# TGoldC/Motion-Planning-for-Autonomous-Driving-with-MPC

Measured on AMD Instinct MI355X. Metric: MPC steps/sec (N=30, nx=6 nu=2) at batch=4096, higher is better.
Workload: dtype f64; 1 GPU; N=30 nx=6 nu=2 bicycle lane-following, batch=4096/GPU, tol 1e-8; mode=converged, gpu=AMD Radeon Graphics

## Files before the change

### motion-planning-for-autonomous-driving-with-mpc_amd/csrc/mpc_solve_plan.h

```cpp
#pragma once
#include <algorithm>
#include <cctype>
#include <cstdlib>
#include <cstring>
#include <string>

#include "mpc_host_common.h"

namespace mpc {

struct Knobs {
    int pipeline, hybrid, hybrid_bx, hybrid_live, pipe_help, pipe_test_abort, pipe_xcd_mask;
    int rescue, rescue_wg, rescue_alone, loop_async, sync_spin, max_batch, friction_lb, bound_mask, big_wg, groups, poison;
    int timing;
    Knobs();
};
enum class KnobParse {
    ON,
    INT,
    FLAG,
    MASK,
    FRIC,
};
struct KnobDef { const char* name; int Knobs::*field; int dflt; KnobParse parse; };
inline constexpr KnobDef KNOBS[] = {
    {"pipeline", &Knobs::pipeline, 1, KnobParse::ON},           {"hybrid", &Knobs::hybrid, 1, KnobParse::INT},
    {"hybrid_bx", &Knobs::hybrid_bx, 0, KnobParse::INT},        {"hybrid_live", &Knobs::hybrid_live, -1, KnobParse::INT},
    {"pipe_help", &Knobs::pipe_help, -1, KnobParse::INT},       {"pipe_test_abort", &Knobs::pipe_test_abort, 0, KnobParse::FLAG},
    {"pipe_xcd_mask", &Knobs::pipe_xcd_mask, 0, KnobParse::MASK}, {"rescue", &Knobs::rescue, 1, KnobParse::ON},
    {"rescue_wg", &Knobs::rescue_wg, 1, KnobParse::INT},        {"rescue_alone", &Knobs::rescue_alone, 0, KnobParse::FLAG},
    {"loop_async", &Knobs::loop_async, 1, KnobParse::ON},       {"sync_spin", &Knobs::sync_spin, 1, KnobParse::ON},
    {"max_batch", &Knobs::max_batch, 0, KnobParse::INT},        {"friction_lb", &Knobs::friction_lb, 0, KnobParse::FRIC},
    {"bound_mask", &Knobs::bound_mask, 1, KnobParse::INT},      {"big_wg", &Knobs::big_wg, 0, KnobParse::FLAG},
    {"groups", &Knobs::groups, 0, KnobParse::INT},              {"poison", &Knobs::poison, 0, KnobParse::FLAG},
    {"timing", &Knobs::timing, 0, KnobParse::INT},
};
inline Knobs::Knobs() { for (const KnobDef& e : KNOBS) this->*e.field = e.dflt; }
inline const KnobDef* find_knob(const char* name) {
    for (const KnobDef& e : KNOBS) if (name && strcmp(name, e.name) == 0) return &e;
    return nullptr;
}
inline int set_knob(Knobs& k, const char* name, const char* value) {
    const KnobDef* e = find_knob(name);
    if (!e) return MPC_ERR_INVALID;
    int v = e->dflt;
    if (value) {
        const long iv = strtol(value, nullptr, 0);
        switch (e->parse) {
            case KnobParse::ON: v = value[0] != '0'; break;
            case KnobParse::INT: v = (int)iv; break;
            case KnobParse::FLAG: v = (value[0] == '\0' ? 1 : (int)iv) != 0; break;
            case KnobParse::MASK: v = (int)(uint32_t)strtoul(value, nullptr, 0); break;
            case KnobParse::FRIC: v = strcmp(value, "ipopt") == 0 ? 1 : strcmp(value, "nlp") == 0 ? 0 : (int)iv; break;
        }
    }
    k.*e->field = v;
    return MPC_OK;
}
// ... 206 lines not shown
```

### motion-planning-for-autonomous-driving-with-mpc_amd/csrc/mpc_stage_math.h

```cpp
#pragma once
#include <math.h>
#include <stdint.h>

#if defined(__HIPCC__)
#define MPC_HD __host__ __device__ __forceinline__
#else
#define MPC_HD inline
#endif

#if defined(__HIP_DEVICE_COMPILE__)
#define MPC_GLOBAL_AS __attribute__((address_space(1)))
#else
#define MPC_GLOBAL_AS
#endif
#define MPC_GP(ptr, idx) (((MPC_GLOBAL_AS __typeof__(*(ptr))*)(ptr))[(uint32_t)(idx)])

namespace mpc {

constexpr double MU_INIT = 0.1, KAPPA_EPS = 10.0, KAPPA_MU = 0.2, THETA_MU = 1.5, TAU_MIN = 0.99;
constexpr double KAPPA_1 = 1e-2, KAPPA_2 = 1e-2, S_MAX = 100.0, KAPPA_SIGMA = 1e10;
constexpr double GAMMA_THETA = 1e-5, GAMMA_PHI = 1e-8, LS_DELTA = 1.0, S_THETA = 1.1, S_PHI = 2.3;
constexpr double ETA_PHI = 1e-8, GAMMA_ALPHA = 0.05;
constexpr double DW_MIN = 1e-20, DW_0 = 1e-4, DW_MAX = 1e40, KW_MINUS = 1.0 / 3.0, KW_PLUS = 8.0, KW_PLUS_BAR = 100.0;
constexpr double SCALING_MAX_GRAD = 100.0;
// ... 185 lines not shown
#define MPC_KX(arr_, R, dk, e) (MB ? MPC_KI(P.M##arr_, R, dk, e) : MPC_K(P.arr_, R, dk, e))
#define MPC_ROWS(expr) [&](int e) -> decltype(auto) { return (expr); }
template <int CNT, class RefFn>
MPC_HD void ws_load_rows(RefFn ref, double* dst) {
#pragma unroll
    for (int i = 0; i + 1 < CNT; i += 2) MPC_LD2(ref(i), dst[i], dst[i + 1]);
    if (CNT & 1) dst[CNT - 1] = ref(CNT - 1);
}
template <int START, int CNT, class RefFn>
MPC_HD void ws_store_run(RefFn ref, const double* src) {
    constexpr int HEAD = START & 1;
    if (HEAD) ref(START) = src[0];
#pragma unroll
    for (int i = HEAD; i + 1 < CNT; i += 2) MPC_ST2(ref(START + i), src[i], src[i + 1]);
    if ((CNT - HEAD) & 1) ref(START + CNT - 1) = src[CNT - 1];
}
template <int CNT, class RefFn>
MPC_HD void ws_store_rows(RefFn ref, const double* src) {
#pragma unroll
    for (int i = 0; i + 1 < CNT; i += 2) MPC_ST2(ref(i), src[i], src[i + 1]);
    if (CNT & 1) ref(CNT - 1) = src[CNT - 1];
}

template <int NX>
struct Dim {
    static constexpr int NU = 2;
    static constexpr int NZ = NX + 2;
    static constexpr int NS = NX * (NX + 1) / 2;
    static constexpr int NH = NX + 5;
    MPC_HD static constexpr int hrow(int i, int j) {
        return i == j ? i : (i == 0 && j == 1) ? NX : (i == 0 && j == 4) ? NX + 1 : (i == 1 && j == 4) ? NX + 2
             : (i == 2 && j == 3) ? NX + 3 : (i == 3 && j == 4) ? NX + 4 : -1;
    }
    static constexpr int B_A = 0, B_RUU = 6, B_GU = 8, B_CN = 10, B_GX = 10 + NX, B_H = 10 + 2 * NX;
    static constexpr int NBLK = NH + 10 + 2 * NX;
    static constexpr int NPK = NS + NX;
    static constexpr int NKK = 2 * NX + 2;
    MPC_HD static constexpr int sidx(int i, int j) { return i * NX - i * (i - 1) / 2 + (j - i); }
};

struct Red0 { double gmax; };
struct Red1 { double a_pr, a_du, dphi; };
struct Red2 { double theta, fcost, logsum, bad; };
struct Red3 { double dual_inf, prim_inf, cmin, cmax, sum_mult, sum_z, theta, fcost, logsum, nan; };

MPC_HD Red0 red_neutral0() { return Red0{0.0}; }
// ... 1538 lines not shown
#pragma unroll
    for (int i = 0; i < NX; ++i) {
        if (i >= NE) { pv[i] = 0.0; continue; }
        double t = s.gx[i] + h[i] + g.G0[i] * kf0 + g.G1[i] * kf1;
        if (i == 2) t += a42 * h[4];
        if (i == 3) { t += a03 * h[0] + a13 * h[1] + a43 * h[4]; if (NE == 6) t += dt * h[NX - 1]; }
        if (i == 4) t += a04 * h[0] + a14 * h[1];
        pv[i] = t;
    }
}

template <int NX>
MPC_HD void ric_store_stage(const PRef& P, uint32_t bb, int k, const double* Ps, const double* pv, const RicGain<NX>& g) {
    using D = Dim<NX>;
    double kk[D::NKK], pk[D::NPK];
#pragma unroll
    for (int j = 0; j < NX; ++j) { kk[j] = g.K0[j]; kk[NX + j] = g.K1[j]; }
    kk[2 * NX] = g.kf0;
    kk[2 * NX + 1] = g.kf1;
#pragma unroll
    for (int i = 0; i < D::NS; ++i) pk[i] = Ps[i];
#pragma unroll
    for (int i = 0; i < NX; ++i) pk[D::NS + i] = pv[i];
    ws_store_rows<D::NKK>(MPC_ROWS(MPC_UK(P.KK, D::NKK, k, e)), kk);
    ws_store_rows<D::NPK>(MPC_ROWS(MPC_UK(P.PK, D::NPK, k, e)), pk);
}

template <int NX, int NE = NX, bool SYM = true>
MPC_HD bool riccati_backward_step(const PRef& P, uint32_t bb, int k, const RicStage<NX>& s, double delta, double hux0,
                                  double hux1, double* Ps, double* pv, bool sym_gk = false) {
    constexpr int NS = Dim<NX>::NS;
    double Pn[NS];
#pragma unroll
    for (int i = 0; i < NS; ++i) Pn[i] = Ps[i];
    RicGain<NX> g;
    if (!ric_matrix_step<NX, NE, SYM>(P, k, s, delta, hux0, hux1, Ps, g, sym_gk)) return false;
    ric_vector_step<NX, NE, SYM>(P, s, Pn, g, pv);
    ric_store_stage<NX>(P, bb, k, Ps, pv, g);
    return true;
}

template <int NX>
MPC_HD bool ric_bwd_any(const PRef& P, uint32_t bb, int k, const RicStage<NX>& s, double delta, double hux0, double hux1,
                        double* Ps, double* pv, bool sym_gk = false) {
    if (NX == 6 && P.dec_s && delta == 0.0) return riccati_backward_step<NX, (NX == 6 ? 5 : NX)>(P, bb, k, s, delta, hux0, hux1, Ps, pv, sym_gk);
    return riccati_backward_step<NX>(P, bb, k, s, delta, hux0, hux1, Ps, pv, sym_gk);
}

// ... 9 lines not shown
        f.K0[j] = MPC_UK(P.KK, D::NKK, k, j);
        f.K1[j] = MPC_UK(P.KK, D::NKK, k, NX + j);
        f.cn[j] = MPC_UK(P.BLK, D::NBLK, k, D::B_CN + j);
    }
    f.kf0 = MPC_UK(P.KK, D::NKK, k, 2 * NX);
    f.kf1 = MPC_UK(P.KK, D::NKK, k, 2 * NX + 1);
#pragma unroll
    for (int i = 0; i < 6; ++i) f.a[i] = MPC_UK(P.BLK, D::NBLK, k, D::B_A + i);
}

template <int NX>
MPC_HD void riccati_forward_step(const PRef& P, uint32_t bb, int k, const FwdStage<NX>& f, double* dx) {
    using D = Dim<NX>;
    const double dt = P.dt;
    double du0 = f.kf0, du1 = f.kf1;
#pragma unroll
    for (int j = 0; j < NX; ++j) { du0 += f.K0[j] * dx[j]; du1 += f.K1[j] * dx[j]; }
    {
        double dz[D::NZ];
        dz[0] = du0;
        dz[1] = du1;
#pragma unroll
        for (int i = 0; i < NX; ++i) dz[2 + i] = dx[i];
        ws_store_rows<D::NZ>(MPC_ROWS(MPC_UK(P.DZ, D::NZ, k, e)), dz);
    }
    double dn[NX];
#pragma unroll
    for (int i = 0; i < NX; ++i) dn[i] = dx[i] - f.cn[i];
    dn[0] += f.a[0] * dx[3] + f.a[1] * dx[4];
    dn[1] += f.a[2] * dx[3] + f.a[3] * dx[4];
    dn[2] += dt * du0;
    dn[3] += dt * du1;
    dn[4] += f.a[4] * dx[2] + f.a[5] * dx[3];
    if (NX == 6) dn[5] += dt * dx[3];
#pragma unroll
    for (int i = 0; i < NX; ++i) dx[i] = dn[i];
}

template <int NX>
MPC_HD void riccati_instance(const PRef& P, int b) {
    using D = Dim<NX>;
    constexpr int NS = D::NS;
    const int N = P.N;
    const uint32_t Bp = (uint32_t)P.Bp, bb = (uint32_t)b;
    if (MPC_U(P.ISC, (uint32_t)IS_STATUS) != ST_RUNNING) return;
    const double dt = P.dt;
    const double delta_last = MPC_U(P.SC, (uint32_t)SC_DLAST);
// ... 203 lines not shown
```

### motion-planning-for-autonomous-driving-with-mpc_amd/csrc/mpcgpu.hip

```cpp
#include <hip/hip_runtime.h>
#include <type_traits>

#include <algorithm>
#include <cctype>
#include <cstdio>
#include <cstdlib>
#include <cstring>
#include <new>
#include <string>
#include <vector>

#include "mpc_host_common.h"
#include "mpc_solve_plan.h"
#include "mpc_closed_loop.h"
#include "mpc_forces_qp.h"
#include "mpc_riccati_mfma.h"
#include "mpc_sens.h"

using namespace mpc;

namespace {

__device__ __forceinline__ void lds_barrier() {
    asm volatile("s_waitcnt lgkmcnt(0)\n\ts_barrier" ::: "memory");
// ... 289 lines not shown
template <int NX, bool INIT, int MAXT, uint32_t VM = 0xFFu>
__global__ void __launch_bounds__(MAXT, (INIT && MAXT <= 256) ? 2 : 1) k_stage(const Params Pk, const int n_mult, const int n_z, const int stash_rows) {
    const PRef P(Pk);
    extern __shared__ __attribute__((aligned(16))) double lds[];
    __shared__ int or_slots[2][8];
    uint32_t blk = blockIdx.x;
    if ((gridDim.x & 7u) == 0u) blk = (blk & 7u) * (gridDim.x >> 3) + (blk >> 3);
    const uint32_t b0 = (blk + (uint32_t)P.tile0 * (64u / (uint32_t)P.bx)) * (uint32_t)P.bx;
    const unsigned long long bits = (!INIT && P.tile_mask != nullptr) ? P.tile_mask[b0 >> 6] : ~0ull;
    stage_block<NX, INIT, MAXT, VM>(P, n_mult, n_z, stash_rows, b0, bits, lds, or_slots);
}

constexpr int32_t HO_IN_MB = 0x40000000;

template <int NCH>
__device__ __forceinline__ void wait_dma_behind(int stages_behind) {
    if (stages_behind >= 4 && 4 * NCH <= 63) asm volatile("s_waitcnt vmcnt(%0)" ::"n"(4 * NCH <= 63 ? 4 * NCH : 0) : "memory");
    else if (stages_behind >= 3 && 3 * NCH <= 63) asm volatile("s_waitcnt vmcnt(%0)" ::"n"(3 * NCH <= 63 ? 3 * NCH : 0) : "memory");
    else if (stages_behind >= 2) asm volatile("s_waitcnt vmcnt(%0)" ::"n"(2 * NCH) : "memory");
    else if (stages_behind == 1) asm volatile("s_waitcnt vmcnt(%0)" ::"n"(NCH) : "memory");
    else asm volatile("s_waitcnt vmcnt(0)" ::: "memory");
}

__device__ __forceinline__ void ho_lists(const PRef& P, const uint32_t bb, int32_t* ho_list, uint32_t* ho_count, const uint32_t* tile_word) {
#if defined(__HIP_DEVICE_COMPILE__)
    const int lane = threadIdx.x & 63;
    const bool active = (int)bb < P.B && (int32_t)MPC_U(P.ISC, (uint32_t)IS_STATUS) == ST_RUNNING;
    if (__ballot(active ? 1 : 0) == 0ull) return;
    const int32_t in_mb = (tile_word != nullptr && (__hip_atomic_load(tile_word + (bb >> 6), __ATOMIC_RELAXED, __HIP_MEMORY_SCOPE_AGENT) >> 31)) ? HO_IN_MB : 0;
    const double e0 = active ? (double)MPC_U(P.SC, (uint32_t)SC_E0) : 0.0;
    const int bucket = e0 >= 1e-3 ? 0 : e0 >= 1e-4 ? 1 : e0 >= 1e-5 ? 2 : 3;
    for (int q = 0; q < (int)HO_BUCKETS; ++q) {
        const unsigned long long mq = __ballot((active && bucket == q) ? 1 : 0);
        if (mq == 0ull) continue;
        uint32_t base = 0u;
        if (lane == 0) base = __hip_atomic_fetch_add(ho_count + q, (uint32_t)__popcll(mq), __ATOMIC_RELAXED, __HIP_MEMORY_SCOPE_AGENT);
        base = (uint32_t)__builtin_amdgcn_readfirstlane((int)base);
        if (active && bucket == q) ho_list[(uint32_t)q * (uint32_t)P.Bp + base + (uint32_t)__popcll(mq & ((1ull << lane) - 1ull))] = (int32_t)bb | in_mb;
    }
#endif
}

template <int NX>
__device__ __forceinline__ unsigned long long riccati_tile(const PRef& P, const uint32_t tile, char* smem, const bool stamp = true, const int handover_live = 0) {
#if defined(__HIP_DEVICE_COMPILE__)
    using D = Dim<NX>;
    constexpr int NS = D::NS;
    constexpr uint32_t BLK_BYTES = MPC_EV(D::NBLK) * 512u;
    constexpr int BLK_CHUNKS = (BLK_BYTES + 1023u) / 1024u;
    constexpr uint32_t SLOT = BLK_CHUNKS * 1024u;
    constexpr int KK_CHUNKS = (D::NKK * 512u + 1023u) / 1024u;
    constexpr int FWD_CHUNKS = KK_CHUNKS + 6;
    constexpr uint32_t FSLOT = FWD_CHUNKS * 1024u;
    static_assert(2 * BLK_CHUNKS <= 63 && RIC_DEPTH == 4 && 4 * FWD_CHUNKS <= 63 && RIC_DEPTH_F == 10, "vmcnt is a 6-bit counter");
    constexpr uint32_t RING_BYTES = (RIC_DEPTH * SLOT > RIC_DEPTH_F * FSLOT) ? RIC_DEPTH * SLOT : RIC_DEPTH_F * FSLOT;
    int* flag = reinterpret_cast<int*>(smem + RING_BYTES);
    const int wave = __builtin_amdgcn_readfirstlane((int)(threadIdx.x >> 6));
    const int lane = threadIdx.x & 63;
    const int b = (int)(tile * 64u) + lane;
    const uint32_t bb = (uint32_t)b;
    const int N = P.N;
    const bool active = (b < P.B) && ((int32_t)MPC_U(P.ISC, (uint32_t)IS_STATUS) == ST_RUNNING);
    const unsigned long long act_mask = __ballot(active ? 1 : 0);
    if (act_mask == 0ull) return 0ull;
    if (__popcll(act_mask) * 64 < handover_live * min(64, P.B - (int)(tile * 64u)) + 64) return 0ull;
#define RIC_STAMP(i) do { if (P.DBG && threadIdx.x == 0 && stamp) P.DBG[blockIdx.x * 16 + (i)] = __builtin_amdgcn_s_memtime(); } while (0)
    RIC_STAMP(0);
    const __amdgpu_buffer_rsrc_t rsrc = P.rws;
    const uint32_t tile_off = tile * P.tile_elems * 8u;
    const uint32_t blk_base = (uint32_t)(uintptr_t)P.BLK - (uint32_t)(uintptr_t)P.WS + tile_off;
    const uint32_t kk_base = (uint32_t)(uintptr_t)P.KK - (uint32_t)(uintptr_t)P.WS + tile_off;
    auto dma = [&](uint32_t src_, uint32_t dst_, int nchunks) {
        const uint32_t src = (uint32_t)__builtin_amdgcn_readfirstlane((int)src_), dst = (uint32_t)__builtin_amdgcn_readfirstlane((int)dst_);
#pragma unroll
        for (int c = 0; c < nchunks; ++c)
        {
            if (P.xcu) __builtin_amdgcn_raw_ptr_buffer_load_lds(rsrc, (lds_ptr_t)(smem + dst + (uint32_t)c * 1024u), 16, lane * 16, (int)(src + (uint32_t)c * 1024u), 0, MPC_AUX_SC1);
            else __builtin_amdgcn_raw_ptr_buffer_load_lds(rsrc, (lds_ptr_t)(smem + dst + (uint32_t)c * 1024u), 16, lane * 16, (int)(src + (uint32_t)c * 1024u), 0, 0);
        }
    };
    auto lds_r = [&](uint32_t off, uint32_t r) { return *reinterpret_cast<const double*>(smem + off + mpc_prow(r) * 8u + (uint32_t)lane * 16u); };
    auto read_stage = [&](uint32_t slot, RicStage<NX>& s) {
#pragma unroll
        for (int i = 0; i < NX; ++i) {
#pragma unroll
            for (int j = i; j < NX; ++j)
                s.H[D::sidx(i, j)] = (D::hrow(i, j) >= 0) ? lds_r(slot, D::B_H + (D::hrow(i, j) >= 0 ? D::hrow(i, j) : 0)) : 0.0;
        }
        s.ruu[0] = lds_r(slot, D::B_RUU);
        s.ruu[1] = lds_r(slot, D::B_RUU + 1);
#pragma unroll
        for (int i = 0; i < 6; ++i) s.a[i] = lds_r(slot, D::B_A + i);
#pragma unroll
        for (int i = 0; i < NX; ++i) { s.gx[i] = lds_r(slot, D::B_GX + i); s.cn[i] = lds_r(slot, D::B_CN + i); }
        s.gu[0] = lds_r(slot, D::B_GU);
        s.gu[1] = lds_r(slot, D::B_GU + 1);
    };
    double delta = 0.0, delta_last = 0.0, hux0 = 0.0, hux1 = 0.0;
    bool need = false, failed = false;
    if (wave == 0) {
        need = active;
        if (active) { delta_last = MPC_U(P.SC, (uint32_t)SC_DLAST); hux0 = MPC_U(P.SC, (uint32_t)SC_HUX0); hux1 = MPC_U(P.SC, (uint32_t)SC_HUX1); }
    }
    for (;;) {
        if (wave >= 2) {
            for (int t = 0; t <= N; ++t) lds_barrier();
        } else if (wave == 1) {
            for (int j = 0; j < RIC_DEPTH - 1 && j <= N; ++j) dma(blk_base + (uint32_t)(N - j) * BLK_BYTES, (uint32_t)j * SLOT, BLK_CHUNKS);
            for (int t = 0; t <= N; ++t) {
                const int k = N - t;
                wait_dma_behind<BLK_CHUNKS>(k < RIC_DEPTH - 2 ? k : RIC_DEPTH - 2);
                lds_barrier();
                const int kn = k - (RIC_DEPTH - 1);
                if (kn >= 0) dma(blk_base + (uint32_t)kn * BLK_BYTES, (uint32_t)((t + RIC_DEPTH - 1) % RIC_DEPTH) * SLOT, BLK_CHUNKS);
            }
        } else {
            bool ok = need;
            const bool sym = delta != 0.0 || delta_last != 0.0;
            auto sweep = [&](auto sym_tag, auto ne_tag) {
                constexpr bool SYM = decltype(sym_tag)::value;
                constexpr int NE = decltype(ne_tag)::value;
                double Ps[NS], pv[NX];
                for (int t = 0; t <= N; ++t) {
                    const int k = N - t;
                    if (t == 15) RIC_STAMP(3);
                    lds_barrier();
                    if (t == 15) RIC_STAMP(4);
                    RicStage<NX> s;
                    read_stage((uint32_t)(t % RIC_DEPTH) * SLOT, s);
                    if (t == 0) {
#pragma unroll
                        for (int i = 0; i < NS; ++i) Ps[i] = s.H[i];
#pragma unroll
                        for (int i = 0; i < NX; ++i) { Ps[D::sidx(i, i)] += delta; pv[i] = s.gx[i]; }
                        if (ok) {
                            double pk[D::NPK];
#pragma unroll
                            for (int i = 0; i < NS; ++i) pk[i] = Ps[i];
#pragma unroll
                            for (int i = 0; i < NX; ++i) pk[NS + i] = pv[i];
                            ws_store_rows<D::NPK>(MPC_ROWS(MPC_UK(P.PK, D::NPK, N, e)), pk);
                        }
                    } else if (ok) {
                        ok = riccati_backward_step<NX, NE, SYM>(P, bb, k, s, delta, hux0, hux1, Ps, pv, SYM && sym);
                    }
                    if (t == 15) RIC_STAMP(5);
                }
            };
            if (__any(sym ? 1 : 0)) sweep(std::true_type{}, std::integral_constant<int, NX>{});
            else if (NX == 6 && P.dec_s) sweep(std::false_type{}, std::integral_constant<int, (NX == 6 ? 5 : NX)>{});
            else sweep(std::false_type{}, std::integral_constant<int, NX>{});
            if (need && ok) need = false;
            else if (need) {
                if (delta == 0.0) delta = (delta_last == 0.0) ? DW_0 : fmax(DW_MIN, KW_MINUS * delta_last);
                else delta *= (delta_last == 0.0) ? KW_PLUS_BAR : KW_PLUS;
                if (delta > DW_MAX) { need = false; failed = true; }
            }
            const int again = __any(need ? 1 : 0);
            asm volatile("s_waitcnt vmcnt(0)" ::: "memory");
            if (lane == 0) *flag = again;
        }
        lds_barrier();
        const int again = lds_uniform(*flag);
        lds_barrier();
        if (!again) break;
    }
    RIC_STAMP(1);
    const bool go = (wave == 0) && active && !failed;
    if (wave >= 3) {
        for (int k = 0; k < N; ++k) lds_barrier();
    } else if (wave >= 1) {
        const int par = wave - 1;
        auto dma_fwd = [&](int k, uint32_t dst) {
            dma(kk_base + (uint32_t)k * (D::NKK * 512u), dst, KK_CHUNKS);
            static_assert(D::B_A % 2 == 0 && D::B_CN % 2 == 0 && D::NKK % 2 == 0, "sub-blocks copied on their own start on a row-pair boundary");
            dma(blk_base + (uint32_t)k * BLK_BYTES + D::B_A * 512u, dst + KK_CHUNKS * 1024u, 3);
            dma(blk_base + (uint32_t)k * BLK_BYTES + D::B_CN * 512u, dst + (KK_CHUNKS + 3) * 1024u, 3);
        };
        for (int j = par; j < RIC_DEPTH_F - 1 && j < N; j += 2) dma_fwd(j, (uint32_t)j * FSLOT);
        for (int k = 0; k < N; ++k) {
            if ((k & 1) == par) {
                const int last = (N - 1 < k + RIC_DEPTH_F - 2) ? N - 1 : k + RIC_DEPTH_F - 2;
                wait_dma_behind<FWD_CHUNKS>((last - k) >> 1);
            }
            lds_barrier();
            const int kn = k + RIC_DEPTH_F - 1;
            if (kn < N && (kn & 1) == par) dma_fwd(kn, (uint32_t)(kn % RIC_DEPTH_F) * FSLOT);
        }
    } else {
        if (active && failed) MPC_U(P.ISC, (uint32_t)IS_STATUS) = P.emit ? ST_SWEEP_FAILED : -7;
        if (go) {
            if (delta > 0.0) MPC_U(P.SC, (uint32_t)SC_DLAST) = delta;
            MPC_U(P.SC, (uint32_t)SC_DELTA) = delta;
        }
        double dx[NX];
#pragma unroll
        for (int i = 0; i < NX; ++i) dx[i] = go ? -(double)MPC_U(P.SC, (uint32_t)(SC_C0 + i)) : 0.0;
        for (int k = 0; k < N; ++k) {
            const uint32_t slot = (uint32_t)(k % RIC_DEPTH_F) * FSLOT;
            if (k == 15) RIC_STAMP(6);
            lds_barrier();
            if (k == 15) RIC_STAMP(7);
            if (k == 0) RIC_STAMP(9);
            FwdStage<NX> f;
#pragma unroll
            for (int j = 0; j < NX; ++j) {
                f.K0[j] = lds_r(slot, (uint32_t)j);
                f.K1[j] = lds_r(slot, (uint32_t)(NX + j));
                f.cn[j] = lds_r(slot + (KK_CHUNKS + 3) * 1024u, (uint32_t)j);
            }
            f.kf0 = lds_r(slot, (uint32_t)(2 * NX));
            f.kf1 = lds_r(slot, (uint32_t)(2 * NX + 1));
#pragma unroll
            for (int i = 0; i < 6; ++i) f.a[i] = lds_r(slot + KK_CHUNKS * 1024u, (uint32_t)i);
            riccati_forward_step<NX>(P, bb, k, f, dx);
            if (k == 15) RIC_STAMP(8);
        }
        if (go) {
            double dz[D::NZ];
            dz[0] = 0.0;
            dz[1] = 0.0;
#pragma unroll
            for (int i = 0; i < NX; ++i) dz[2 + i] = dx[i];
            ws_store_rows<D::NZ>(MPC_ROWS(MPC_UK(P.DZ, D::NZ, N, e)), dz);
        }
    }
    RIC_STAMP(2);
#undef RIC_STAMP
    return act_mask;
#else
    return 0ull;
#endif
}

template <int NX>
__global__ void __launch_bounds__(192) k_riccati(const Params Pk) {
    const PRef P(Pk);
    extern __shared__ __attribute__((aligned(16))) char smem[];
    const uint32_t tile = blockIdx.x + (uint32_t)P.tile0;
    const unsigned long long act_mask = riccati_tile<NX>(P, tile, smem);
    if (P.tile_mask != nullptr && threadIdx.x == 0) P.tile_mask[tile] = act_mask;
}

struct PipeArgs {
    uint32_t* ctl;
    uint32_t ntiles;
    uint32_t xcd_mask;
    uint32_t n_ric;
    uint32_t cap;
    uint32_t items;
    uint32_t handover;
    int32_t* ho_list;
    uint32_t flags;
};
constexpr uint32_t PIPE_EXIT = 0xFFFFFFFFu;
constexpr unsigned long long PIPE_SPIN_LIMIT = 5000000ull;
#ifndef MPC_PIPE_SLEEP
#define MPC_PIPE_SLEEP 8
#endif

__device__ __forceinline__ void pipe_acquire() {
#if defined(__HIP_DEVICE_COMPILE__)
    __builtin_amdgcn_fence(__ATOMIC_ACQUIRE, "workgroup");
// ... 69 lines not shown
                if (t == 0) {
                    uint32_t ok = 1u;
                    const uint32_t need = A.items * round;
                    const unsigned long long t0 = wall_clock64();
                    while (pipe_ld(stage_done + tile) < need) {
                        if (pipe_ld(abort_w)) { ok = 0u; break; }
                        if (wall_clock64() - t0 > PIPE_SPIN_LIMIT) {
                            pipe_st(abort_w + 28, (tile << 16) | (round & 0xFFFFu)); pipe_st(abort_w + 29, pipe_ld(stage_done + tile)); pipe_st(abort_w + 31, (uint32_t)(wall_clock64() - t0));
                            const unsigned long long t1 = wall_clock64();
                            while (wall_clock64() - t1 < 100000ull) __builtin_amdgcn_s_sleep(8);
                            pipe_st(abort_w + 30, pipe_ld(stage_done + tile));
                            pipe_st(abort_w, 2u); ok = 0u; break;
                        }
                        __builtin_amdgcn_s_sleep(MPC_PIPE_SLEEP);
                    }
                    waited += wall_clock64() - t0;
                    pipe_acquire();
                    asm volatile("s_waitcnt vmcnt(0)" ::: "memory");
                    sh_word[1] = ok;
                }
                lds_barrier();
                if (lds_uniform(sh_word[1]) == 0u) return;
                PIPE_STAMP(12);
                const unsigned long long mask = riccati_tile<NX>(P, tile, reinterpret_cast<char*>(lds), n_pass == 5u, (int)A.handover);
                if (mask == 0ull) {
                    fin |= 1u << j;
                    if (t == 0) {
                        if (round > 0u && P.mbw_live > 0 && __popcll(__hip_atomic_load(P.tile_mask + tile, __ATOMIC_RELAXED, __HIP_MEMORY_SCOPE_AGENT)) <= P.mbw_live)
                        {   __hip_atomic_fetch_or(stage_done + tile, 0x80000000u, __ATOMIC_RELAXED, __HIP_MEMORY_SCOPE_AGENT);
                            asm volatile("s_waitcnt vmcnt(0)" ::: "memory");
                        }
                        atomicMax(A.ctl + PIPE_ABORT + 1, round);
                        pipe_add(X + 48, 1u);
                    }
                } else if (t < 64) {
                    if (t == 0) __hip_atomic_store(P.tile_mask + tile, mask, __ATOMIC_RELAXED, __HIP_MEMORY_SCOPE_AGENT);
                    asm volatile("s_waitcnt vmcnt(0)" ::: "memory");
                    if (t == 0) {
                        const uint32_t tk = pipe_add(X + 32, A.items);
                        for (uint32_t q = 0; q < A.items; ++q)
                            __hip_atomic_store(slots + ((tk + q) & (A.cap - 1u)), ((unsigned long long)(tk + q + 1u) << 32) | (unsigned long long)((tile << 8) | q),
                                               __ATOMIC_RELAXED, __HIP_MEMORY_SCOPE_AGENT);
                    }
                }
                PIPE_STAMP(13);
                ++n_pass;
                lds_barrier();
                if constexpr (helper) if (mask != 0ull) {
                    if (t == 0) {
                        uint32_t item = PIPE_EXIT;
                        unsigned long long bits = 0ull;
                        uint32_t jn = j, rn = round;
                        do { if (++jn == n_own) { jn = 0u; ++rn; } } while (((fin >> jn) & 1u) && jn != j);
                        const uint32_t tile_n = (slot + jn * n_ric) * n_xcd + xcd;
                        if (pipe_ld(stage_done + tile_n) < A.items * rn) {
                            uint32_t hd = pipe_ld(X + 16);
                            bool got = false;
                            while ((int32_t)(pipe_ld(X + 32) - hd) > 0) {
                                uint32_t seen = hd;
                                if (__hip_atomic_compare_exchange_strong(X + 16, &seen, hd + 1u, __ATOMIC_RELAXED, __ATOMIC_RELAXED, __HIP_MEMORY_SCOPE_AGENT)) { got = true; break; }
                                hd = seen;
                            }
                            if (got) {
                                const unsigned long long* sl = slots + (hd & (A.cap - 1u));
                                const unsigned long long t0 = wall_clock64();
                                for (;;) {
                                    const unsigned long long v = __hip_atomic_load(sl, __ATOMIC_RELAXED, __HIP_MEMORY_SCOPE_AGENT);
                                    if ((uint32_t)(v >> 32) == hd + 1u) { item = (uint32_t)v; break; }
                                    if (pipe_ld(abort_w)) break;
                                    if (wall_clock64() - t0 > PIPE_SPIN_LIMIT) { pipe_st(abort_w + 28, hd); pipe_st(abort_w + 29, pipe_ld(X + 32)); pipe_st(abort_w + 31, (uint32_t)(wall_clock64() - t0)); pipe_st(abort_w, 3u); break; }
// ... 1524 lines not shown
    N_SCRATCH
};

struct mpc_handle {
    HostProblem hp;
    std::string err;
    int device = 0;
    size_t cap_Bp = 0;
    bool ws_mailbox = false;
    double* d_ws = nullptr;
    int32_t* d_iws = nullptr;
    double *d_LB = nullptr, *d_UB = nullptr;
    unsigned long long* d_tile_mask = nullptr;
    double* d_state = nullptr;
    size_t cap_state = 0;
    size_t tile_mask_cap = 0;
    uint32_t* d_pipe = nullptr;
    int pipe_flip = 0;
    size_t pipe_clean[2] = {0, 0};
    size_t pipe_words = 0;
    uint32_t* h_pipe = nullptr;
    bool pipe_disabled = false;
    int pipe_aborts = 0;
    static constexpr int PIPE_ABORTS_MAX = 3;
    int last_mode = 0;
    int32_t* d_counter = nullptr;
    int32_t* h_counter = nullptr;
    hipEvent_t ev_poll[4][2] = {};
    size_t cap_io = 0;
    double *d_x0 = nullptr, *d_p = nullptr, *d_xout = nullptr, *d_kkt = nullptr;
    int32_t *d_status = nullptr, *d_iters = nullptr;
    hipStream_t own_stream = nullptr;
    hipStream_t sub_stream[MAX_GROUPS] = {nullptr, nullptr, nullptr, nullptr};
    hipEvent_t ev_fork = nullptr, ev_join[MAX_GROUPS] = {nullptr, nullptr, nullptr, nullptr};
    bool profiling = false;
    bool prof_span = false;
    double prof[6] = {0, 0, 0, 0, 0, 0};
    double res_prof[8] = {0, 0, 0, 0, 0, 0, 0, 0};
    double pipe_prof[8] = {0, 0, 0, 0, 0, 0, 0, 0};
    int n_cu = 256;
    uint32_t xcd_mask = 0xFFu;
    std::vector<hipEvent_t> ev_pool;
    uint32_t* d_fail = nullptr;
    bool async_loop = false;
    bool async_ok = false;
    uint32_t* h_fail = nullptr;
// ... 177 lines not shown
    return MPC_OK;
}

int mpc_set_profiling(mpc_handle* h, int32_t enable) {
    if (!h) return MPC_ERR_INVALID;
    h->profiling = enable != 0;
    h->prof_span = enable == 2;
    return MPC_OK;
}

int mpc_set_option(mpc_handle* h, const char* name, const char* value) {
    if (!h || !name) return MPC_ERR_INVALID;
    const int rc = set_knob(h->knobs, name, value);
    if (rc) h->err = std::string("unknown option (or a value this build does not support): ") + name;
    else apply_fric_literal(h->hp, h->knobs.friction_lb);
    return rc;
}

int mpc_get_option(const mpc_handle* h, const char* name, int64_t* value) {
    if (!h || !name || !value) return MPC_ERR_INVALID;
    long v = 0;
    if (std::string(name) == "pipe_disabled") { *value = h->pipe_disabled ? 1 : 0; return MPC_OK; }
    if (std::string(name) == "pipe_aborts") { *value = h->pipe_aborts; return MPC_OK; }
    const int rc = get_knob(h->knobs, name, &v);
    if (rc == MPC_OK) *value = (int64_t)v;
    return rc;
}

int mpc_last_rescued(const mpc_handle* h) { return h ? h->rescued_last : MPC_ERR_INVALID; }

int mpc_get_pipeline_profile(const mpc_handle* h, double out[8]) {
    if (!h || !out) return MPC_ERR_INVALID;
    for (int i = 0; i < 8; ++i) out[i] = h->pipe_prof[i];
    return MPC_OK;
}

int mpc_get_resident_profile(const mpc_handle* h, double out[8]) {
    if (!h || !out) return MPC_ERR_INVALID;
    for (int i = 0; i < 8; ++i) out[i] = h->res_prof[i];
    return MPC_OK;
}

int mpc_measure_copy_bandwidth(mpc_handle* h, size_t bytes, int32_t reps, double* gbs) {
    if (!h || !gbs || reps < 1 || bytes < (1u << 20)) return MPC_ERR_INVALID;
    HIP_TRY(h, hipSetDevice(h->device));
    const size_t n = bytes / 16;
// ... 440 lines not shown
            h->async_ok = true;
            return MPC_OK;
        }
        HIP_TRY(h, wait_stream(h, stream));
        h->h_fail[0] = h->h_pipe[14];
        for (int q = 0; q < 4; ++q) h->h_fail[2 + q] = h->h_pipe[16 + q];
        if (h->resc_ran && !in_rescue) h->rescued_last = (int)h->h_pipe[20];
        report_wg_trace(d_wtrace, n_wtrace);
        if (P.DBG) {
            rc = report_wg_timing(h, P.DBG, pl.wg_grid);
            if (rc) return rc;
            P.DBG = nullptr;
        }
        piped = true;
        it = (int)h->h_fail[2];
        h->res_prof[1] = 1; h->res_prof[2] = it; h->res_prof[3] = pl.wg_grid; h->res_prof[4] = h->h_fail[3]; h->res_prof[5] = h->h_fail[4]; h->res_prof[6] = h->h_fail[5];
    } else if (pl.pipe_path) {
        PipeArgs A;
        A.ntiles = (uint32_t)ntiles;
        A.n_ric = (uint32_t)pl.n_ric;
        A.xcd_mask = pl.xcd_mask;
        A.items = 64u / (uint32_t)bx;
        A.cap = pl.pipe_cap;
        A.flags = kn.pipe_test_abort ? 2u : 0u;
        A.handover = (uint32_t)hand;
        A.ho_list = nullptr;
        if (hand > 0) {
            A.ho_list = static_cast<int32_t*>(scratch_get(h, SCR_HO_LIST, (size_t)HO_BUCKETS * Bp * sizeof(int32_t)));
            if (!A.ho_list) { h->err = "out of device memory"; return MPC_ERR_HIP; }
        }
        A.ctl = ctl;
        unsigned long long* d_pdbg = nullptr;
        if (pl.pipe_timing) {
            HIP_TRY(h, hipMalloc(&t_pdbg.p, sizeof(unsigned long long) * 16 * (size_t)h->n_cu));
            d_pdbg = t_pdbg.as<unsigned long long>();
            HIP_TRY(h, hipMemsetAsync(d_pdbg, 0, sizeof(unsigned long long) * 16 * (size_t)h->n_cu, stream));
            P.DBG = d_pdbg;
        }
        prof.next(3, stream);
        P.mbw_live = pl.mbw_live;
        const size_t lds_pipe = std::max(pl.lds_bytes, pl.ric_lds);
        if (pl.pipe_help) hipLaunchKernelGGL((k_pipeline<NX, 2, true>), dim3(h->n_cu), dim3(threads), lds_pipe, stream, P, A, h->hp.n_mult, h->hp.n_z, stash_rows);
        else if (pl.masked) hipLaunchKernelGGL((k_pipeline<NX, 2>), dim3(h->n_cu), dim3(threads), lds_pipe, stream, P, A, h->hp.n_mult, h->hp.n_z, stash_rows);
        else hipLaunchKernelGGL((k_pipeline<NX, false>), dim3(h->n_cu), dim3(threads), lds_pipe, stream, P, A, h->hp.n_mult, h->hp.n_z, stash_rows);
        if (hand <= 0) prof.end(stream);
        if (hand > 0) {
            if (!h->prof_span) prof.next(5, stream);
            wg_list = A.ho_list; wg_list_n = ctl + PIPE_HO;
            launch_wg((const uint32_t*)(ctl + PIPE_ABORT), ctl + PIPE_WG, h->async_loop ? nullptr : ctl + PIPE_ABORT);
        }
        prof.end(stream);
        if (h->async_loop) {
            hipLaunchKernelGGL(k_loop_sticky, dim3(1), dim3(1), 0, stream, (const uint32_t*)(ctl + PIPE_ABORT), h->d_fail + 1);
            HIP_TRY(h, hipGetLastError());
            h->async_ok = true;
            h->last_mode = 1;
            return MPC_OK;
        }
        if (hand <= 0) HIP_TRY(h, hipMemcpyAsync(h->h_pipe, ctl + PIPE_ABORT, PIPE_FIN_WORDS * sizeof(uint32_t), hipMemcpyDeviceToHost, stream));
        HIP_TRY(h, wait_stream(h, stream));
        h->h_fail[0] = h->h_pipe[14];
        report_wg_trace(d_wtrace, n_wtrace);
        for (int q = 0; q < 4; ++q) h->h_fail[2 + q] = h->h_pipe[16 + q];
        if (h->resc_ran && !in_rescue) h->rescued_last = (int)h->h_pipe[20];
        if (hand > 0) {
            h->res_prof[1] = 1; h->res_prof[2] = h->h_fail[2]; h->res_prof[3] = pl.wg_grid;
            h->res_prof[4] = h->h_fail[3]; h->res_prof[5] = h->h_fail[4]; h->res_prof[6] = h->h_fail[5];
        }
        if (h->h_pipe[0] != 0u) {
            h->pipe_disabled = true;
            h->resc_in_kernel = h->resc_ran = false;
            fprintf(stderr, "[mpcgpu] single-launch pipeline abandoned (bounded wait expired: code %u, %u / %u, a millisecond later %u, waited %u ticks); re-running with one launch per kernel\n",
                    h->h_pipe[0], h->h_pipe[28], h->h_pipe[29], h->h_pipe[30], h->h_pipe[31]);
            report_arrivals(ctl, ntiles, A.items);
            const int rc_again = solve_dev_impl<NX>(h, B, d_x0, d_p, d_obst, d_x_out, d_status, d_iters, d_kkt, stream, trace, trace_rows, n_it_out, in_rescue);
            if (++h->pipe_aborts < mpc_handle::PIPE_ABORTS_MAX) h->pipe_disabled = false;
            return rc_again;
        }
        P.DBG = nullptr;
        if (d_pdbg) { rc = report_pipe_timing(h, d_pdbg); if (rc) return rc; }
        piped = true;
        h->last_mode = 1;
        it = (int)h->h_pipe[1];
        const unsigned long long* st64 = reinterpret_cast<const unsigned long long*>(h->h_pipe + 2);
        h->pipe_prof[1] = 1; h->pipe_prof[2] = it;
        h->pipe_prof[3] = (double)st64[0] * 1e-5; h->pipe_prof[4] = (double)st64[1] * 1e-5; h->pipe_prof[5] = (double)st64[2] * 1e-5;
        h->pipe_prof[6] = (double)st64[3]; h->pipe_prof[7] = (double)h->h_pipe[12] + 1e-3 * (double)h->h_pipe[13];
    }
    if (!piped) {
        if (!h->async_loop) HIP_TRY(h, hipMemsetAsync(h->d_fail, 0, sizeof(uint32_t), stream));
        if (pl.polled) HIP_TRY(h, hipMemsetAsync(h->d_counter, 0, sizeof(int32_t) * MAX_GROUPS * MAX_POLL_IT, stream));
        if (G > 1) {
            HIP_TRY(h, hipEventRecord(h->ev_fork, stream));
// ... 754 lines not shown
```

Baseline: 5.328 million MPC steps/s.

## Replace per-stage workgroup barriers in Riccati sweeps with LDS progress counters

Removes the lock-step lds_barrier calls between the DMA loader waves and the compute wave in the backward and forward Riccati sweeps. In their place each wave publishes progress words in LDS and waits on them with a bounded spin, so idle waves no longer take part in the barriers. It also switches the workspace row stores to raw buffer stores with immediate offsets. The bounded wait adds an abort path, reported through the existing pipeline-abandon mechanism, and a test knob that forces it to expire; the risks are spin overhead and spurious timeouts.

Result: slower. 4.585 million MPC steps/s (-13.9%).

```diff
diff --git a/motion-planning-for-autonomous-driving-with-mpc_amd/csrc/mpc_solve_plan.h b/motion-planning-for-autonomous-driving-with-mpc_amd/csrc/mpc_solve_plan.h
--- a/motion-planning-for-autonomous-driving-with-mpc_amd/csrc/mpc_solve_plan.h
+++ b/motion-planning-for-autonomous-driving-with-mpc_amd/csrc/mpc_solve_plan.h
@@ -10,7 +10,7 @@
 namespace mpc {
 
 struct Knobs {
-    int pipeline, hybrid, hybrid_bx, hybrid_live, pipe_help, pipe_test_abort, pipe_xcd_mask;
+    int pipeline, hybrid, hybrid_bx, hybrid_live, pipe_help, pipe_test_abort, pipe_test_expire, pipe_xcd_mask;
     int rescue, rescue_wg, rescue_alone, loop_async, sync_spin, max_batch, friction_lb, bound_mask, big_wg, groups, poison;
     int timing;
     Knobs();
@@ -33,7 +33,7 @@
     {"max_batch", &Knobs::max_batch, 0, KnobParse::INT},        {"friction_lb", &Knobs::friction_lb, 0, KnobParse::FRIC},
     {"bound_mask", &Knobs::bound_mask, 1, KnobParse::INT},      {"big_wg", &Knobs::big_wg, 0, KnobParse::FLAG},
     {"groups", &Knobs::groups, 0, KnobParse::INT},              {"poison", &Knobs::poison, 0, KnobParse::FLAG},
-    {"timing", &Knobs::timing, 0, KnobParse::INT},
+    {"timing", &Knobs::timing, 0, KnobParse::INT},              {"pipe_test_expire", &Knobs::pipe_test_expire, 0, KnobParse::FLAG},
 };
 inline Knobs::Knobs() { for (const KnobDef& e : KNOBS) this->*e.field = e.dflt; }
 inline const KnobDef* find_knob(const char* name) {
diff --git a/motion-planning-for-autonomous-driving-with-mpc_amd/csrc/mpc_stage_math.h b/motion-planning-for-autonomous-driving-with-mpc_amd/csrc/mpc_stage_math.h
--- a/motion-planning-for-autonomous-driving-with-mpc_amd/csrc/mpc_stage_math.h
+++ b/motion-planning-for-autonomous-driving-with-mpc_amd/csrc/mpc_stage_math.h
@@ -231,6 +231,32 @@
     if (CNT & 1) ref(CNT - 1) = src[CNT - 1];
 }
 
+#if defined(__HIP_DEVICE_COMPILE__)
+template <int CNT, class RefFn>
+__device__ __forceinline__ void ws_store_rows_imm(RefFn ref, const double* src) {
+    const WsRefD r0 = ref(0);
+    const __amdgpu_buffer_rsrc_t d = r0.P.rws;
+    const uint32_t uni = (uint32_t)mpc_uni(r0.aoff + r0.uoff);
+#pragma unroll
+    for (int g = 0; g < CNT; g += 8) {
+        uint32_t base = r0.voff + (uint32_t)mpc_uni(uni + (uint32_t)g * 512u);
+        asm volatile("" : "+v"(base));
+#pragma unroll
+        for (int i = g; i < g + 8 && i < CNT; i += 2) {
+            if (i + 1 < CNT) {
+                const mpc_v2u a = __builtin_bit_cast(mpc_v2u, src[i]), b = __builtin_bit_cast(mpc_v2u, src[i + 1]);
+                __builtin_amdgcn_raw_buffer_store_b128(mpc_v4u{a.x, a.y, b.x, b.y}, d, (int)(base + (uint32_t)(i - g) * 512u), 0, 0);
+            } else {
+                __builtin_amdgcn_raw_buffer_store_b64(__builtin_bit_cast(mpc_v2u, src[i]), d, (int)(base + (uint32_t)(i - g) * 512u), 0, 0);
+            }
+        }
+    }
+}
+#else
+template <int CNT, class RefFn>
+MPC_HD void ws_store_rows_imm(RefFn ref, const double* src) { ws_store_rows<CNT>(ref, src); }
+#endif
+
 template <int NX>
 struct Dim {
     static constexpr int NU = 2;
@@ -1815,8 +1841,8 @@
     for (int i = 0; i < D::NS; ++i) pk[i] = Ps[i];
 #pragma unroll
     for (int i = 0; i < NX; ++i) pk[D::NS + i] = pv[i];
-    ws_store_rows<D::NKK>(MPC_ROWS(MPC_UK(P.KK, D::NKK, k, e)), kk);
-    ws_store_rows<D::NPK>(MPC_ROWS(MPC_UK(P.PK, D::NPK, k, e)), pk);
+    ws_store_rows_imm<D::NKK>(MPC_ROWS(MPC_UK(P.KK, D::NKK, k, e)), kk);
+    ws_store_rows_imm<D::NPK>(MPC_ROWS(MPC_UK(P.PK, D::NPK, k, e)), pk);
 }
 
 template <int NX, int NE = NX, bool SYM = true>
@@ -1872,7 +1898,7 @@
         dz[1] = du1;
 #pragma unroll
         for (int i = 0; i < NX; ++i) dz[2 + i] = dx[i];
-        ws_store_rows<D::NZ>(MPC_ROWS(MPC_UK(P.DZ, D::NZ, k, e)), dz);
+        ws_store_rows_imm<D::NZ>(MPC_ROWS(MPC_UK(P.DZ, D::NZ, k, e)), dz);
     }
     double dn[NX];
 #pragma unroll
diff --git a/motion-planning-for-autonomous-driving-with-mpc_amd/csrc/mpcgpu.hip b/motion-planning-for-autonomous-driving-with-mpc_amd/csrc/mpcgpu.hip
--- a/motion-planning-for-autonomous-driving-with-mpc_amd/csrc/mpcgpu.hip
+++ b/motion-planning-for-autonomous-driving-with-mpc_amd/csrc/mpcgpu.hip
@@ -335,6 +335,33 @@
     else asm volatile("s_waitcnt vmcnt(0)" ::: "memory");
 }
 
+constexpr int RIC_W_LD = 0, RIC_W_CP = 2, RIC_W_QUIT = 3, RIC_WORDS = 4;
+constexpr unsigned long long RIC_SPIN_LIMIT = 5000000ull;
+enum : int { RIC_QUIT_BWD = 1, RIC_QUIT_FWD = 2, RIC_QUIT_LOADER = 3, RIC_QUIT_TEST = 4 };
+__device__ __forceinline__ int ric_peek(const int* w) { return *reinterpret_cast<const volatile int*>(w); }
+__device__ __forceinline__ void ric_publish(int* w, const int v) {
+    asm volatile("" ::: "memory");
+    if ((threadIdx.x & 63) == 0) *reinterpret_cast<volatile int*>(w) = v;
+}
+__device__ __forceinline__ bool ric_wait(const int* w, const int need, const int seen, int* quit, const int code, const bool expire_now = false) {
+    bool ok = true;
+    if (lds_uniform(seen) < need || expire_now) {
+        const unsigned long long t0 = wall_clock64();
+        for (;;) {
+            if (!expire_now && lds_uniform(ric_peek(w)) >= need) break;
+            if (lds_uniform(ric_peek(quit)) != 0) { ok = false; break; }
+            if (expire_now || wall_clock64() - t0 > RIC_SPIN_LIMIT) {
+                if ((threadIdx.x & 63) == 0) *reinterpret_cast<volatile int*>(quit) = expire_now ? (int)RIC_QUIT_TEST : code;
+                ok = false;
+                break;
+            }
+            __builtin_amdgcn_s_sleep(1);
+        }
+    }
+    asm volatile("" ::: "memory");
+    return ok;
+}
+
 __device__ __forceinline__ void ho_lists(const PRef& P, const uint32_t bb, int32_t* ho_list, uint32_t* ho_count, const uint32_t* tile_word) {
 #if defined(__HIP_DEVICE_COMPILE__)
     const int lane = threadIdx.x & 63;
@@ -355,7 +382,8 @@
 }
 
 template <int NX>
-__device__ __forceinline__ unsigned long long riccati_tile(const PRef& P, const uint32_t tile, char* smem, const bool stamp = true, const int handover_live = 0) {
+__device__ __forceinline__ unsigned long long riccati_tile(const PRef& P, const uint32_t tile, char* smem, uint32_t& gave_up, const bool stamp = true, const int handover_live = 0,
+                                                          const bool test_expire = false) {
 #if defined(__HIP_DEVICE_COMPILE__)
     using D = Dim<NX>;
     constexpr int NS = D::NS;
@@ -368,6 +396,8 @@
     static_assert(2 * BLK_CHUNKS <= 63 && RIC_DEPTH == 4 && 4 * FWD_CHUNKS <= 63 && RIC_DEPTH_F == 10, "vmcnt is a 6-bit counter");
     constexpr uint32_t RING_BYTES = (RIC_DEPTH * SLOT > RIC_DEPTH_F * FSLOT) ? RIC_DEPTH * SLOT : RIC_DEPTH_F * FSLOT;
     int* flag = reinterpret_cast<int*>(smem + RING_BYTES);
+    int* prog = flag + 1;
+    gave_up = 0u;
     const int wave = __builtin_amdgcn_readfirstlane((int)(threadIdx.x >> 6));
     const int lane = threadIdx.x & 63;
     const int b = (int)(tile * 64u) + lane;
@@ -379,6 +409,8 @@
     if (__popcll(act_mask) * 64 < handover_live * min(64, P.B - (int)(tile * 64u)) + 64) return 0ull;
 #define RIC_STAMP(i) do { if (P.DBG && threadIdx.x == 0 && stamp) P.DBG[blockIdx.x * 16 + (i)] = __builtin_amdgcn_s_memtime(); } while (0)
     RIC_STAMP(0);
+    if (threadIdx.x < (unsigned)RIC_WORDS) prog[threadIdx.x] = 0;
+    lds_barrier();
     const __amdgpu_buffer_rsrc_t rsrc = P.rws;
     const uint32_t tile_off = tile * P.tile_elems * 8u;
     const uint32_t blk_base = (uint32_t)(uintptr_t)P.BLK - (uint32_t)(uintptr_t)P.WS + tile_off;
@@ -417,15 +449,17 @@
     }
     for (;;) {
         if (wave >= 2) {
-            for (int t = 0; t <= N; ++t) lds_barrier();
         } else if (wave == 1) {
             for (int j = 0; j < RIC_DEPTH - 1 && j <= N; ++j) dma(blk_base + (uint32_t)(N - j) * BLK_BYTES, (uint32_t)j * SLOT, BLK_CHUNKS);
             for (int t = 0; t <= N; ++t) {
                 const int k = N - t;
                 wait_dma_behind<BLK_CHUNKS>(k < RIC_DEPTH - 2 ? k : RIC_DEPTH - 2);
-                lds_barrier();
+                ric_publish(prog + RIC_W_LD, t + 1);
                 const int kn = k - (RIC_DEPTH - 1);
-                if (kn >= 0) dma(blk_base + (uint32_t)kn * BLK_BYTES, (uint32_t)((t + RIC_DEPTH - 1) % RIC_DEPTH) * SLOT, BLK_CHUNKS);
+                if (kn >= 0) {
+                    if (!ric_wait(prog + RIC_W_CP, t, ric_peek(prog + RIC_W_CP), prog + RIC_W_QUIT, RIC_QUIT_LOADER)) break;
+                    dma(blk_base + (uint32_t)kn * BLK_BYTES, (uint32_t)((t + RIC_DEPTH - 1) % RIC_DEPTH) * SLOT, BLK_CHUNKS);
+                }
             }
         } else {
             bool ok = need;
@@ -434,13 +468,16 @@
                 constexpr bool SYM = decltype(sym_tag)::value;
                 constexpr int NE = decltype(ne_tag)::value;
                 double Ps[NS], pv[NX];
+                int seen = lds_uniform(ric_peek(prog + RIC_W_LD));
                 for (int t = 0; t <= N; ++t) {
                     const int k = N - t;
                     if (t == 15) RIC_STAMP(3);
-                    lds_barrier();
+                    if (!ric_wait(prog + RIC_W_LD, t + 1, seen, prog + RIC_W_QUIT, RIC_QUIT_BWD, test_expire && t == 1)) break;
                     if (t == 15) RIC_STAMP(4);
+                    const int seen_v = ric_peek(prog + RIC_W_LD);
                     RicStage<NX> s;
                     read_stage((uint32_t)(t % RIC_DEPTH) * SLOT, s);
+                    seen = lds_uniform(seen_v);
                     if (t == 0) {
 #pragma unroll
                         for (int i = 0; i < NS; ++i) Ps[i] = s.H[i];
@@ -452,12 +489,13 @@
                             for (int i = 0; i < NS; ++i) pk[i] = Ps[i];
 #pragma unroll
                             for (int i = 0; i < NX; ++i) pk[NS + i] = pv[i];
-                            ws_store_rows<D::NPK>(MPC_ROWS(MPC_UK(P.PK, D::NPK, N, e)), pk);
+                            ws_store_rows_imm<D::NPK>(MPC_ROWS(MPC_UK(P.PK, D::NPK, N, e)), pk);
                         }
                     } else if (ok) {
                         ok = riccati_backward_step<NX, NE, SYM>(P, bb, k, s, delta, hux0, hux1, Ps, pv, SYM && sym);
                     }
                     if (t == 15) RIC_STAMP(5);
+                    ric_publish(prog + RIC_W_CP, t + 1);
                 }
             };
             if (__any(sym ? 1 : 0)) sweep(std::true_type{}, std::integral_constant<int, NX>{});
@@ -475,13 +513,16 @@
         }
         lds_barrier();
         const int again = lds_uniform(*flag);
+        gave_up = (uint32_t)lds_uniform(ric_peek(prog + RIC_W_QUIT));
+        if (gave_up) break;
+        if (threadIdx.x < (unsigned)RIC_W_QUIT) prog[threadIdx.x] = 0;
         lds_barrier();
         if (!again) break;
     }
+    if (gave_up) { asm volatile("s_waitcnt vmcnt(0)" ::: "memory"); return act_mask; }
     RIC_STAMP(1);
     const bool go = (wave == 0) && active && !failed;
     if (wave >= 3) {
-        for (int k = 0; k < N; ++k) lds_barrier();
     } else if (wave >= 1) {
         const int par = wave - 1;
         auto dma_fwd = [&](int k, uint32_t dst) {
@@ -495,10 +536,13 @@
             if ((k & 1) == par) {
                 const int last = (N - 1 < k + RIC_DEPTH_F - 2) ? N - 1 : k + RIC_DEPTH_F - 2;
                 wait_dma_behind<FWD_CHUNKS>((last - k) >> 1);
-            }
-            lds_barrier();
+                ric_publish(prog + RIC_W_LD + par, k + 1);
+            }
             const int kn = k + RIC_DEPTH_F - 1;
-            if (kn < N && (kn & 1) == par) dma_fwd(kn, (uint32_t)(kn % RIC_DEPTH_F) * FSLOT);
+            if (kn < N && (kn & 1) == par) {
+                if (!ric_wait(prog + RIC_W_CP, k, ric_peek(prog + RIC_W_CP), prog + RIC_W_QUIT, RIC_QUIT_LOADER)) break;
+                dma_fwd(kn, (uint32_t)(kn % RIC_DEPTH_F) * FSLOT);
+            }
         }
     } else {
         if (active && failed) MPC_U(P.ISC, (uint32_t)IS_STATUS) = P.emit ? ST_SWEEP_FAILED : -7;
@@ -509,12 +553,14 @@
         double dx[NX];
 #pragma unroll
         for (int i = 0; i < NX; ++i) dx[i] = go ? -(double)MPC_U(P.SC, (uint32_t)(SC_C0 + i)) : 0.0;
+        int seen = lds_uniform(ric_peek(prog + RIC_W_LD));
         for (int k = 0; k < N; ++k) {
             const uint32_t slot = (uint32_t)(k % RIC_DEPTH_F) * FSLOT;
             if (k == 15) RIC_STAMP(6);
-            lds_barrier();
+            if (!ric_wait(prog + RIC_W_LD + (k & 1), k + 1, seen, prog + RIC_W_QUIT, RIC_QUIT_FWD)) break;
             if (k == 15) RIC_STAMP(7);
             if (k == 0) RIC_STAMP(9);
+            const int seen_v = ric_peek(prog + RIC_W_LD + ((k + 1) & 1));
             FwdStage<NX> f;
 #pragma unroll
             for (int j = 0; j < NX; ++j) {
@@ -526,8 +572,10 @@
             f.kf1 = lds_r(slot, (uint32_t)(2 * NX + 1));
 #pragma unroll
             for (int i = 0; i < 6; ++i) f.a[i] = lds_r(slot + KK_CHUNKS * 1024u, (uint32_t)i);
+            seen = lds_uniform(seen_v);
             riccati_forward_step<NX>(P, bb, k, f, dx);
             if (k == 15) RIC_STAMP(8);
+            ric_publish(prog + RIC_W_CP, k + 1);
         }
         if (go) {
             double dz[D::NZ];
@@ -535,11 +583,14 @@
             dz[1] = 0.0;
 #pragma unroll
             for (int i = 0; i < NX; ++i) dz[2 + i] = dx[i];
-            ws_store_rows<D::NZ>(MPC_ROWS(MPC_UK(P.DZ, D::NZ, N, e)), dz);
+            ws_store_rows_imm<D::NZ>(MPC_ROWS(MPC_UK(P.DZ, D::NZ, N, e)), dz);
         }
     }
     RIC_STAMP(2);
 #undef RIC_STAMP
+    lds_barrier();
+    gave_up = (uint32_t)lds_uniform(ric_peek(prog + RIC_W_QUIT));
+    if (gave_up) asm volatile("s_waitcnt vmcnt(0)" ::: "memory");
     return act_mask;
 #else
     return 0ull;
@@ -551,7 +602,12 @@
     const PRef P(Pk);
     extern __shared__ __attribute__((aligned(16))) char smem[];
     const uint32_t tile = blockIdx.x + (uint32_t)P.tile0;
-    const unsigned long long act_mask = riccati_tile<NX>(P, tile, smem);
+    uint32_t gave_up;
+    const unsigned long long act_mask = riccati_tile<NX>(P, tile, smem, gave_up);
+    if (gave_up && threadIdx.x < 64) {
+        const uint32_t bb = tile * 64u + threadIdx.x;
+        if ((act_mask >> threadIdx.x) & 1ull) MPC_U(P.ISC, (uint32_t)IS_STATUS) = P.emit ? ST_SWEEP_FAILED : -7;
+    }
     if (P.tile_mask != nullptr && threadIdx.x == 0) P.tile_mask[tile] = act_mask;
 }
 
@@ -667,7 +723,12 @@
                 lds_barrier();
                 if (lds_uniform(sh_word[1]) == 0u) return;
                 PIPE_STAMP(12);
-                const unsigned long long mask = riccati_tile<NX>(P, tile, reinterpret_cast<char*>(lds), n_pass == 5u, (int)A.handover);
+                uint32_t gave_up;
+                const unsigned long long mask = riccati_tile<NX>(P, tile, reinterpret_cast<char*>(lds), gave_up, n_pass == 5u, (int)A.handover, (A.flags & 4u) != 0u);
+                if (gave_up) {
+                    if (t == 0) { pipe_st(abort_w + 28, (tile << 16) | (round & 0xFFFFu)); pipe_st(abort_w + 29, gave_up); pipe_st(abort_w + 30, 0u); pipe_st(abort_w + 31, 0u); pipe_st(abort_w, 5u); }
+                    return;
+                }
                 if (mask == 0ull) {
                     fin |= 1u << j;
                     if (t == 0) {
@@ -690,7 +751,7 @@
                 }
                 PIPE_STAMP(13);
                 ++n_pass;
-                lds_barrier();
+                if (mask == 0ull) lds_barrier();
                 if constexpr (helper) if (mask != 0ull) {
                     if (t == 0) {
                         uint32_t item = PIPE_EXIT;
@@ -2261,6 +2322,7 @@
     uint32_t* h_pipe = nullptr;
     bool pipe_disabled = false;
     int pipe_aborts = 0;
+    int pipe_abort_code = 0;
     static constexpr int PIPE_ABORTS_MAX = 3;
     int last_mode = 0;
     int32_t* d_counter = nullptr;
@@ -2484,6 +2546,7 @@
     long v = 0;
     if (std::string(name) == "pipe_disabled") { *value = h->pipe_disabled ? 1 : 0; return MPC_OK; }
     if (std::string(name) == "pipe_aborts") { *value = h->pipe_aborts; return MPC_OK; }
+    if (std::string(name) == "pipe_abort_code") { *value = h->pipe_abort_code; return MPC_OK; }
     const int rc = get_knob(h->knobs, name, &v);
     if (rc == MPC_OK) *value = (int64_t)v;
     return rc;
@@ -2970,7 +3033,7 @@
         A.xcd_mask = pl.xcd_mask;
         A.items = 64u / (uint32_t)bx;
         A.cap = pl.pipe_cap;
-        A.flags = kn.pipe_test_abort ? 2u : 0u;
+        A.flags = (kn.pipe_test_abort ? 2u : 0u) | (kn.pipe_test_expire ? 4u : 0u);
         A.handover = (uint32_t)hand;
         A.ho_list = nullptr;
         if (hand > 0) {
@@ -3017,6 +3080,7 @@
         }
         if (h->h_pipe[0] != 0u) {
             h->pipe_disabled = true;
+            h->pipe_abort_code = (int)h->h_pipe[0];
             h->resc_in_kernel = h->resc_ran = false;
             fprintf(stderr, "[mpcgpu] single-launch pipeline abandoned (bounded wait expired: code %u, %u / %u, a millisecond later %u, waited %u ticks); re-running with one launch per kernel\n",
                     h->h_pipe[0], h->h_pipe[28], h->h_pipe[29], h->h_pipe[30], h->h_pipe[31]);
```
